# LuisaGroup/LuisaRender

Hardware: AMD Instinct MI355X
Metric: Msamples/s (+ fraction of HBM roofline) at fixed SPP, 1/2/4/8 GPU (higher is better)
Workload: dtype f32; 1 GPU; Contemporary Bathroom-class (procedural stand-in, ~600k tris), 1024x1024, 1024spp, depth 16; integrator=MegaPath, sampler=Independent (seed 19980810), spp=1024, parallelism=single GPU, collective=none (single GPU), scheduler=path pool, two contexts per lane (megapool_kernel.h)

## Files before the change

### __graft_entry__.py

```python
import os
import subprocess
import sys

ROOT = os.path.dirname(os.path.abspath(__file__))
if ROOT not in sys.path:
    sys.path.insert(0, ROOT)


def build() -> None:
    jobs = f"-j{min(os.cpu_count() or 4, 16)}"
    subprocess.check_call(["make", "-C", ROOT, jobs, "host", "oracle", "hip", "cli", "ieee", "shallow", "noearly", "nopair", "noride"])
    if os.path.isdir("/root/reference/src"):
        subprocess.check_call(["make", "-C", ROOT, jobs, "ref"])
    import luisarender_amd
    from luisarender_amd import _ffi
    _ffi.host_lib()
    assert os.path.exists(os.path.join(ROOT, "luisarender_amd", "lib", "liblrhip.so"))


def smoke() -> None:
    import numpy as np
    from luisarender_amd import Scene
    from oracle.check import Oracle
    from luisarender_amd.render import MegaPathRenderer
    from luisarender_amd.scenes import cornell_box

    scene = Scene.from_string(cornell_box(resolution=64, spp=8))
    renderer = MegaPathRenderer(0)
    renderer.upload(scene)
    renderer.render(0, 8, counters=True, sync=True)
    gpu = renderer.download(converted=False)
    cpu, counters = Oracle(scene).render(0, 8)
    rel = float(np.abs(gpu[..., :3] - cpu[..., :3]).sum() / np.abs(cpu[..., :3]).sum())
    gc = renderer.counters()
# ... 11 lines not shown
```

### include/lrhip.h

```cpp
#ifndef LRHIP_H
#define LRHIP_H

#include "lr_scene.h"

#ifdef __cplusplus
extern "C" {
#endif

typedef struct lrhip_ctx lrhip_ctx;

#define LRHIP_OK 0
#define LRHIP_ERROR_INVALID (-1)
#define LRHIP_ERROR_DEVICE (-2)
#define LRHIP_ERROR_UNSUPPORTED (-3)

typedef struct lrhip_render_params {
    uint32_t spp_begin, spp_end;
    uint32_t tile_begin, tile_end, tile_stride;
    uint32_t flags;
    uint32_t balance_shards;
    float shutter_weight;
} lrhip_render_params;

#define LRHIP_RENDER_COUNTERS 1u
// ... 102 lines not shown
int lrhip_set_wavefront(lrhip_ctx *ctx, uint32_t mode, uint32_t slice_paths);

#define LRHIP_FEAT_POOL 4096u
int lrhip_set_scheduler(lrhip_ctx *ctx, uint32_t mode);
int lrhip_set_texture_storage(lrhip_ctx *ctx, uint32_t mode);
uint64_t lrhip_packed_texels(lrhip_ctx *ctx);

uint32_t lrhip_pool_auto_triangles(uint32_t max_depth, uint32_t scene_spp);

#define LRHIP_FAMILY_NONE 0u
#define LRHIP_FAMILY_LANE 1u
#define LRHIP_FAMILY_POOL 2u
#define LRHIP_FAMILY_WAVEFRONT 3u
#define LRHIP_FAMILY_AOV 4u
#define LRHIP_PLAN_FLAG_COUNTERS 1u
#define LRHIP_PLAN_FLAG_ENV_TREE 2u
#define LRHIP_PLAN_FLAG_PACKED_TEXELS 4u
#define LRHIP_PLAN_FLAG_WANTS_POOL 8u
#define LRHIP_PLAN_FLAG_FIXED_FITS 16u
#define LRHIP_PLAN_WORDS 8
int lrhip_plan_kernels(uint32_t features, uint32_t force_features, uint32_t flags, uint32_t sampler_kind, uint32_t wf_mode, uint32_t max_depth,
                       uint32_t out[LRHIP_PLAN_WORDS]);

const char *lrhip_last_error(void);

#ifdef __cplusplus
}
#endif
#endif
```

### luisarender_amd/_ffi.py

```python
from __future__ import annotations

import ctypes as C
import os

_ROOT = os.path.dirname(os.path.abspath(__file__))
REPO_ROOT = os.path.dirname(_ROOT)
LIB_DIR = os.path.join(_ROOT, "lib")

u32, u64, i32, f32 = C.c_uint32, C.c_uint64, C.c_int32, C.c_float


class Vertex(C.Structure):
    _fields_ = [(n, f32) for n in ("px", "py", "pz", "nx", "ny", "nz", "u", "v")]


class Triangle(C.Structure):
    _fields_ = [("i0", u32), ("i1", u32), ("i2", u32)]


class AliasEntry(C.Structure):
    _fields_ = [("prob", f32), ("alias", u32)]


class UInt4(C.Structure):
# ... 203 lines not shown
        lib.lrhip_film_download.argtypes = [C.c_void_p, C.c_void_p, C.c_int]
        lib.lrhip_get_counters.argtypes = [C.c_void_p, C.POINTER(HipCounters)]
        lib.lrhip_last_render_ms.restype = C.c_double
        lib.lrhip_last_render_ms.argtypes = [C.c_void_p]
        lib.lrhip_set_stream.argtypes = [C.c_void_p, C.c_void_p]
        lib.lrhip_last_variant.restype = C.c_uint32
        lib.lrhip_last_variant.argtypes = [C.c_void_p]
        lib.lrhip_set_diagnostics.argtypes = [C.c_void_p, C.c_uint32, C.c_double]
        lib.lrhip_set_wavefront.argtypes = [C.c_void_p, C.c_uint32, C.c_uint32]
        lib.lrhip_set_scheduler.argtypes = [C.c_void_p, C.c_uint32]
        lib.lrhip_set_texture_storage.argtypes = [C.c_void_p, C.c_uint32]
        lib.lrhip_packed_texels.restype = C.c_uint64
        lib.lrhip_packed_texels.argtypes = [C.c_void_p]
        lib.lrhip_aov_download.argtypes = [C.c_void_p, C.c_uint32, C.c_void_p]
        lib.lrhip_denoise_default_params.restype = None
        lib.lrhip_denoise_default_params.argtypes = [C.POINTER(DenoiseParams)]
        lib.lrhip_denoise.argtypes = [C.c_void_p, C.POINTER(DenoiseParams)] + [C.c_void_p] * 5
        lib.lrhip_aov_denoise.argtypes = [C.c_void_p, C.POINTER(DenoiseParams), C.c_uint32, C.c_uint32, C.c_void_p]
        lib.lrhip_last_denoise_ms.restype = C.c_double
        lib.lrhip_last_denoise_ms.argtypes = [C.c_void_p]
        lib.lrhip_trace_rays.argtypes = [C.c_void_p, C.POINTER(RayQueryParams)]
        lib.lrhip_last_trace_ms.restype = C.c_double
        lib.lrhip_last_trace_ms.argtypes = [C.c_void_p]
        lib._lr_ready = True
    return lib
```

### luisarender_amd/csrc/hip/dev_scene.h

```cpp
#pragma once
#include "../../../include/lr_scene.h"
#include "dev_math.h"

namespace lrd {

struct alignas(16) DInstance {
    uint32_t handle[4];
    float c0[3]; uint32_t vertex_offset;
    float c1[3]; uint32_t triangle_offset;
    float c2[3]; uint32_t pad0;
    float t[3];  uint32_t pad1;
    float n0[3]; uint32_t pad2;
    float n1[3]; uint32_t pad3;
    float n2[3]; uint32_t pad4;
};
static_assert(sizeof(DInstance) == 128, "DInstance must be one cache line");

struct alignas(16) DClosure {
    uint32_t kind;
    uint32_t dynamic;
    float alpha_x, alpha_y;
    float c0[3]; float s0;
    float c1[3]; float s1;
    float c2[3]; float s2;
// ... 51 lines not shown
    const float *pdf;
    float direction[3];
    float cos_half_angle;
    uint32_t visible, constant_emission;
    uint32_t kind;
    float child_scale[2];
    uint32_t tree;
    const DEnvironment *child[2];
};

enum : uint32_t { kEnvNone = 0u, kEnvConstant = 1u, kEnvImage = 2u, kEnvDirectional = 3u, kEnvCombined = 4u };

struct DShadeTri {
    float p0[3];  uint32_t flags;
    float e1[3];  uint32_t tags;
    float e2[3];  uint32_t offset_bits;
    float n0[3];  float uv0x;
    float n1[3];  float uv0y;
    float n2[3];  float uv1x;
    float uv1y, uv2x, uv2y, tri_pdf;
    uint32_t inst, prim, tri_offset, pad;
};
static_assert(sizeof(DShadeTri) == 128, "one line per triangle");

constexpr uint32_t kWfKinds = 3u;
constexpr uint32_t kWfHeavyWords = 14u;
constexpr uint32_t kWfContWords = 25u;
constexpr uint32_t kWfSamplerWordsMax = 4u;
#ifndef LR_WF_ITEM
#define LR_WF_ITEM 1024
#endif
constexpr uint32_t kWfItemRecords = LR_WF_ITEM;
enum : uint32_t { kWfCountHeavy = 0u, kWfCountCont = 3u, kWfWorkCont = 4u, kWfWorkHeavy = 5u, kWfCounterWords = 8u,
                  kWfCarry = 8u, kWfCounterBufferWords = 12u };
struct WfArgs {
    uint32_t *heavy;
    uint32_t *cont;
    uint32_t *counts;
    uint32_t capacity;
    unsigned long long *accum;
    float accum_scale;
    uint32_t count_at_flush;
};

struct DScene {
    const DNodeQ *nodes;
// ... 19 lines not shown
    const lr_medium *media;
    uint32_t env_medium_tag;
    uint32_t integrator_kind, integrator_flags;
    float rr_threshold, env_prob;
    uint32_t light_count;
    uint32_t has_lights;
    uint32_t sampler_kind, seed;
    float film_clamp;
    uint32_t sampler_spp;
    uint32_t sobol_scale;
    float shutter_weight;
    uint32_t sampler_tile;
    uint32_t sampler_tile_jitter;
    const uint32_t *sobol_matrices;
    const uint32_t *sobol_bytes;
    const uint64_t *vdc_sobol, *vdc_sobol_inv;
    const uint64_t *vdc_bytes, *vdc_inv_bytes;
    const DEnvironment *env;
    WfArgs wf;
    float *aov;
    float *aov_partial;
    uint32_t aov_channels;
    uint32_t aov_offset[LR_AOV_COMPONENTS];
};

typedef const DScene __attribute__((address_space(4))) *DScenePtr;

struct DCounters {
    unsigned long long paths, closest_rays, shadow_rays, nodes_visited, tris_tested, surface_hits, nee_samples,
        path_length_sum, trace_steps, trace_steps_busy, shade_calls, shade_busy, trace_steps_starved, shade_cycles, trace_cycles, wave_cycles, nodes_empty,
        shade_light_cycles, shade_closure_cycles, shade_regen_cycles;
    unsigned long long probe[16];
};

struct RenderArgs {
    float4 *film;
    uint32_t spp_begin, spp_end;
    uint32_t tile_begin, tile_end, tile_stride;
    uint32_t tiles_x, tiles_y;
    uint32_t chunk_count;
    uint32_t item_count;
    uint32_t *work_counter;
    float4 *partial;
    uint32_t *spill;
    uint32_t total_threads;
    DCounters *counters;
// ... 32 lines not shown
```

### luisarender_amd/csrc/hip/dev_shade.h

```cpp
#pragma once
#include "dev_bsdf.h"
#include "dev_trace.h"

namespace lrd {


LR_HD uint32_t xxhash32_4(uint32_t x, uint32_t y, uint32_t z, uint32_t w) {
    constexpr uint32_t P2 = 2246822519u, P3 = 3266489917u, P4 = 668265263u, P5 = 374761393u;
    auto rot = [](uint32_t h) { return (h << 17u) | (h >> 15u); };
    auto h = w + P5 + x * P3;
    h = P4 * rot(h);
    h += y * P3;
    h = P4 * rot(h);
    h += z * P3;
    h = P4 * rot(h);
    h = P2 * (h ^ (h >> 15u));
    h = P3 * (h ^ (h >> 13u));
    return h ^ (h >> 16u);
}

LR_HD uint32_t xxhash32_1(uint32_t p) {
    constexpr uint32_t P2 = 2246822519u, P3 = 3266489917u, P4 = 668265263u, P5 = 374761393u;
    auto h = p + P5;
    h = P4 * ((h << 17u) | (h >> 15u));
// ... 582 lines not shown
    sp.tags = h.y;
    sp.offset_bits = h.w;
    sp.tri_offset = tri_offset;
    sp.uv = (sp.flags & LR_SHAPE_HAS_VERTEX_UV) ?
                f2{bary.x * uv0.x + bary.y * uv1.x + bary.z * uv2.x, bary.x * uv0.y + bary.y * uv1.y + bary.z * uv2.y} :
                f2{bary.y, bary.z};
    if (FULL) {
        auto r0 = ip[5], r1 = ip[6], r2 = ip[7];
        f3 n0 = mk3(a0.w, a1.x, a1.y), n1 = mk3(b0.w, b1.x, b1.y), n2 = mk3(c0.w, c1.x, c1.y);
        auto ns_local = bary.x * n0 + bary.y * n1 + bary.z * n2;
        f2 duv0{uv1.x - uv0.x, uv1.y - uv0.y}, duv1{uv2.x - uv0.x, uv2.y - uv0.y};
        auto det = duv0.x * duv1.y - duv0.y * duv1.x;
        auto inv_det = 1.f / det;
        auto dpdu_local = (dp0 * duv1.y - dp1 * duv0.y) * inv_det;
        auto fallback = frame_from_normal(sp.ng);
        auto dpdu = det == 0.f ? fallback.s : mul(dpdu_local);
        auto ns = (sp.flags & LR_SHAPE_HAS_VERTEX_NORMAL) ?
                      normalize(mk3(r0.x, r0.y, r0.z) * ns_local.x + mk3(r1.x, r1.y, r1.z) * ns_local.y + mk3(r2.x, r2.y, r2.z) * ns_local.z) :
                      sp.ng;
        sp.shading = frame_from_normal_tangent(face_forward(ns, sp.ng), dpdu);
    }
}

LR_D void reconstruct_baked(const DScene &scene, uint32_t tri, float u, float v, SurfacePoint &sp) {
    auto q = reinterpret_cast<const float4 *>(scene.shade_tris + tri);
    auto q0 = q[0], q1 = q[1], q2 = q[2], q3 = q[3], q4 = q[4], q5 = q[5], q6 = q[6];
    auto w = 1.f - u - v;
    f3 p0 = mk3(q0.x, q0.y, q0.z), e1 = mk3(q1.x, q1.y, q1.z), e2 = mk3(q2.x, q2.y, q2.z);
    sp.p = p0 + e1 * u + e2 * v;
    auto c = cross(e1, e2);
    sp.area = length(c) * .5f;
    sp.ng = normalize(c);
    sp.flags = __float_as_uint(q0.w);
    sp.tags = __float_as_uint(q1.w);
    sp.offset_bits = __float_as_uint(q2.w);
    sp.tri_offset = reinterpret_cast<const uint32_t *>(scene.shade_tris + tri)[30];
    f2 uv0{q3.w, q4.w}, uv1{q5.w, q6.x}, uv2{q6.y, q6.z};
    sp.uv = (sp.flags & LR_SHAPE_HAS_VERTEX_UV) ? f2{w * uv0.x + u * uv1.x + v * uv2.x, w * uv0.y + u * uv1.y + v * uv2.y} : f2{u, v};
    f2 duv0{uv1.x - uv0.x, uv1.y - uv0.y}, duv1{uv2.x - uv0.x, uv2.y - uv0.y};
    auto det = duv0.x * duv1.y - duv0.y * duv1.x;
    auto inv_det = 1.f / det;
    auto fallback = frame_from_normal(sp.ng);
    auto dpdu = det == 0.f ? fallback.s : (e1 * duv1.y - e2 * duv0.y) * inv_det;
    auto ns = (sp.flags & LR_SHAPE_HAS_VERTEX_NORMAL) ?
                  normalize(mk3(q3.x, q3.y, q3.z) * w + mk3(q4.x, q4.y, q4.z) * u + mk3(q5.x, q5.y, q5.z) * v) :
                  sp.ng;
    sp.shading = frame_from_normal_tangent(face_forward(ns, sp.ng), dpdu);
}



LR_D float surface_opacity(const DScene &scene, uint32_t tag, f2 uv) {
    auto one = [&](uint32_t t) {
        auto alpha_tex = scene.surfaces[t].raw.alpha_tex;
        return alpha_tex >= 0 ? texture_eval(scene, alpha_tex, uv).x : 1.f;
    };
    if (scene.surfaces[tag].raw.kind != LR_SURFACE_MIX) { return one(tag); }
    uint32_t stack[8];
    auto sp = 0u;
    stack[sp++] = tag;
    auto opacity = 1.f;
    while (sp > 0u) {
        const auto tag_here = stack[--sp];
        auto &s = scene.surfaces[tag_here].raw;
        if (s.kind == LR_SURFACE_MIX && sp + 2u <= 8u) { stack[sp++] = s.u[1], stack[sp++] = s.u[0]; }
        else { opacity *= one(tag_here); }
    }
    return opacity;
}

// ... 61 lines not shown
    auto n = front ? sp.ng : -sp.ng;
    return offset_ray_origin(sp.p, intersection_offset_factor(sp.offset_bits) * n);
}

LR_D void light_evaluate_with(const DScene &scene, const SurfacePoint &lp, float tri_pdf, f3 p_from, f3 &L, float &pdf);
LR_D void light_evaluate(const DScene &scene, const SurfacePoint &lp, uint32_t prim, f3 p_from, f3 &L, float &pdf) {
    light_evaluate_with(scene, lp, scene.tri_pdf[lp.tri_offset + prim], p_from, L, pdf);
}
LR_D void light_evaluate_with(const DScene &scene, const SurfacePoint &lp, float tri_pdf, f3 p_from, f3 &L, float &pdf) {
    auto &light = scene.lights[lp.tags & 4095u];
    auto pdf_area = tri_pdf / lp.area;
    auto cos_wo = abs_dot(normalize(p_from - lp.p), lp.ng);
    f3 Le = mk3(light.L[0], light.L[1], light.L[2]);
    if (light.dynamic) {
        auto v = texture_eval(scene, light.emission_tex, lp.uv);
        Le = max0(mk3(v.x, v.y, v.z)) * light.scale;
    }
    auto diff = lp.p - p_from;
    auto p = dot(diff, diff) * pdf_area * (1.0f / cos_wo);
    auto invalid = fabsf(cos_wo) < 1e-6f || (!light.two_sided && lp.back_facing);
    L = invalid ? mk3(0.f) : Le;
    pdf = invalid ? 0.f : p;
}


LR_D f3 mul3(const float *m, f3 v) { return mk3(m[0], m[1], m[2]) * v.x + mk3(m[3], m[4], m[5]) * v.y + mk3(m[6], m[7], m[8]) * v.z; }

struct EnvTables {
    const lr_texture *textures;
    const float *texels;
};
struct EnvEval {
    f3 L;
    float pdf;
};
struct EnvSample {
    f3 wi, L;
    float pdf;
};

LR_D f3 env_radiance(const EnvTables &tb, const DEnvironment &env, f2 uv) {
    auto v = texture_eval_tables(tb.textures, tb.texels, env.emission_tex, uv);
    auto rgb = env.constant_emission ? extend_rgb(v, tb.textures[env.emission_tex].channels) : mk3(v.x, v.y, v.z);
    return max0(rgb);
}
LR_D float env_directional_pdf(float p, float theta) {
    float sn, cs;
// ... 172 lines not shown
        return;
    }
    auto sa = env.child_scale[0], sb = env.child_scale[1];
    auto weight_a = sa / (sa + sb);
    auto first = u.x < weight_a;
    u.x = first ? u.x / weight_a : (u.x - weight_a) / (1.f - weight_a);
    auto s = env_sample_one(tb, env.child[first ? 0 : 1], u);
    auto o = env_evaluate_one(tb, env.child[first ? 1 : 0], s.wi);
    if (first) {
        L = s.L * sa + o.L * sb;
        pdf = lerp(s.pdf, o.pdf, 1.f - weight_a);
    } else {
        L = o.L * sa + s.L * sb;
        pdf = lerp(o.pdf, s.pdf, 1.f - weight_a);
    }
    wi = normalize(mul3(env.env_to_world, s.wi));
}

struct LightPick {
    Ray shadow;
    f3 L;
    float pdf;
};
template<bool ENV, bool NULL_SHAPE = false>
LR_D LightPick sample_one_light(const DScene &scene, const SurfacePoint &it, float u_light_selection, f2 u_light_surface) {
    LightPick out;
    out.L = mk3(0.f), out.pdf = 0.f;
    auto n = static_cast<float>(scene.light_count);
    auto is_env = false;
    auto tag = 0u;
    auto prob = 0.f;
    if (scene.env_prob == 1.f) {
        is_env = true, prob = 1.f;
    } else if (scene.env_prob == 0.f) {
        tag = static_cast<uint32_t>(clampf(u_light_selection * n, 0.f, n - 1.f)), prob = 1.f / n;
    } else {
        auto uu = (u_light_selection - scene.env_prob) / (1.f - scene.env_prob);
        tag = static_cast<uint32_t>(clampf(uu * n, 0.f, n - 1.f));
        is_env = u_light_selection < scene.env_prob;
        prob = is_env ? scene.env_prob : (1.f - scene.env_prob) / n;
    }
    if (is_env) {
        f3 wi;
        if (ENV && scene.env_kind != kEnvConstant) {
            env_sample(scene, u_light_surface, wi, out.L, out.pdf);
            out.pdf *= prob;
        } else {
            auto z = 1.0f - 2.0f * u_light_surface.x;
            auto r = sqrtf(fmaxf(1.0f - z * z, 0.0f));
            float sn, cs;
            sincos_2pi(u_light_surface.y, sn, cs);
            auto w = mk3(r * cs, r * sn, z);
            auto e = scene.env_to_world;
            wi = normalize(mk3(e[0], e[1], e[2]) * w.x + mk3(e[3], e[4], e[5]) * w.y + mk3(e[6], e[7], e[8]) * w.z);
            out.L = mk3(scene.env_L[0], scene.env_L[1], scene.env_L[2]);
            out.pdf = (kInvPi * 0.25f) * prob;
        }
        out.shadow.o = NULL_SHAPE ? it.p : robust_origin(it, wi);
        out.shadow.d = wi;
        out.shadow.t_min = 0.f, out.shadow.t_max = kFloatMax;
    } else {
        auto handle = scene.light_instances[tag];
        auto lh = reinterpret_cast<const uint4 *>(scene.instances + handle.instance_id)[0];
        auto l_tri_offset = scene.instances[handle.instance_id].triangle_offset;
        float u_remapped;
        auto slot = alias_slot(u_light_surface.x, lh.z, u_remapped);
        auto entry = scene.tri_alias[l_tri_offset + slot];
        auto pick = alias_pick(entry.prob, entry.alias, slot, u_remapped);
        f2 ut{pick.u, u_light_surface.y};
        f2 uvt = ut.x < ut.y ? f2{0.5f * ut.x, -0.5f * ut.x + ut.y} : f2{-0.5f * ut.y + ut.x, 0.5f * ut.y};
        SurfacePoint lp;
        reconstruct<false>(scene, handle.instance_id, pick.index, mk3(uvt.x, uvt.y, 1.0f - uvt.x - uvt.y), lp);
        lp.back_facing = dot(lp.ng, it.p - lp.p) < 0.f;
        light_evaluate(scene, lp, pick.index, it.p, out.L, out.pdf);
        out.pdf *= prob;
        auto p_from = NULL_SHAPE ? it.p : robust_origin(it, lp.p - it.p);
        auto Lv = lp.p - p_from;
        auto dist = length(Lv);
        out.shadow.o = p_from;
        out.shadow.d = Lv * (1.f / dist);
        out.shadow.t_min = 0.f, out.shadow.t_max = dist * .9999f;
    }
    return out;
// ... 4 lines not shown
```

### luisarender_amd/csrc/hip/lrhip_internal.h

```cpp
#pragma once
#include "../../../include/lrhip.h"

#include <hip/hip_runtime.h>

#include <algorithm>
#include <cmath>
#include <cstddef>
#include <cstring>
#include <string>
#include <vector>

#include "megapath_kernel.h"
#include "megapool_kernel.h"
#include "variants.h"

namespace lrh {

int fail(int code, const std::string &msg);

#define LR_HIP_CHECK(expr)                                                                                   \
    do {                                                                                                     \
        auto err_ = (expr);                                                                                  \
        if (err_ != hipSuccess) {                                                                            \
            return lrh::fail(LRHIP_ERROR_DEVICE, std::string{#expr} + ": " + hipGetErrorString(err_));       \
// ... 98 lines not shown
    hipEvent_t denoise_begin{nullptr}, denoise_end{nullptr};
    bool denoise_timed{false};
    lrh::DeviceBuffer raycast_rays, raycast_out;
    hipEvent_t raycast_begin{nullptr}, raycast_end{nullptr};
    double raycast_ms{0.};
    bool raycast_pending{false};
    int raycast_blocks[2]{-1, -1};
};

namespace lrh {

int kernel_blocks(lrhip_ctx *ctx, const KernelEntry &entry, unsigned lds_bytes, uint32_t &blocks_per_cu);

void release_scene(lrhip_ctx *ctx);

std::string validate_indices(const lr_scene *s);
constexpr uint64_t kByteTextureFloatBytes = 192ull << 20u;
std::vector<uint32_t> pack_byte_textures(const lr_scene *s, std::vector<lr_texture> &textures);
uint32_t bvh_depth(const lr_accel &accel);
std::vector<lrd::DNodeQ> build_packed_nodes(const lr_scene *s);
std::vector<uint8_t> build_padded_triangles(const lr_scene *s);
std::vector<lrd::DInstance> build_instances(const lr_scene *s);
std::vector<lrd::DShadeTri> build_shade_tris(const lr_scene *s, const std::vector<lrd::DInstance> &instances, std::string &error);
void set_camera(lrd::DScene &d, const lr_scene *s);

struct Chunking {
    uint32_t count, big_count, big, small;
};
Chunking chunking_of(uint32_t spp, double shard_tiles, double item_scale, bool taper);
int fixed_point_bits(float film_clamp, float shutter_weight, uint32_t spp);
int ensure_accum(lrhip_ctx *ctx, uint32_t pixel_count);
int ensure_pool(lrhip_ctx *ctx, uint32_t resident_blocks);
int render_wavefront(lrhip_ctx *ctx, const lrhip_render_params *p, const KernelPlan &plan, uint32_t tiles_x, uint32_t tiles_y,
                     uint32_t tiles_in_range, uint32_t tile_count);

hipError_t launch_resolve_partial(lrhip_ctx *ctx, const float4 *partial, uint32_t chunk_count, uint32_t tiles_x, uint32_t tile_begin,
                                  uint32_t tile_end, uint32_t tile_stride);
hipError_t launch_resolve_aov_partial(lrhip_ctx *ctx, uint32_t chunk_count, uint32_t tiles_x, uint32_t tile_begin, uint32_t tile_end,
                                      uint32_t tile_stride);
hipError_t launch_wf_resolve(lrhip_ctx *ctx, double inv_scale);
hipError_t launch_wf_carry(lrhip_ctx *ctx, uint32_t margin, uint32_t mode);

}
```

### luisarender_amd/csrc/hip/lrhip_tables.hip

```cpp
#include "lrhip_internal.h"

#include <limits>

namespace lrh {

namespace {
void normal_matrix(const float *m, float out[9]) {
    float a[3][3];
    for (auto c = 0; c < 3; c++) {
        for (auto r = 0; r < 3; r++) { a[c][r] = m[c * 4 + r]; }
    }
    auto one_over_det = 1.0f / (a[0][0] * (a[1][1] * a[2][2] - a[2][1] * a[1][2]) -
                                a[1][0] * (a[0][1] * a[2][2] - a[2][1] * a[0][2]) +
                                a[2][0] * (a[0][1] * a[1][2] - a[1][1] * a[0][2]));
    float inv[3][3];
    inv[0][0] = (a[1][1] * a[2][2] - a[2][1] * a[1][2]) * one_over_det;
    inv[0][1] = (a[2][1] * a[0][2] - a[0][1] * a[2][2]) * one_over_det;
    inv[0][2] = (a[0][1] * a[1][2] - a[1][1] * a[0][2]) * one_over_det;
    inv[1][0] = (a[2][0] * a[1][2] - a[1][0] * a[2][2]) * one_over_det;
    inv[1][1] = (a[0][0] * a[2][2] - a[2][0] * a[0][2]) * one_over_det;
    inv[1][2] = (a[1][0] * a[0][2] - a[0][0] * a[1][2]) * one_over_det;
    inv[2][0] = (a[1][0] * a[2][1] - a[2][0] * a[1][1]) * one_over_det;
    inv[2][1] = (a[2][0] * a[0][1] - a[0][0] * a[2][1]) * one_over_det;
    inv[2][2] = (a[0][0] * a[1][1] - a[1][0] * a[0][1]) * one_over_det;
// ... 106 lines not shown
        const lr_vertex *v[3] = {s->vertices + mesh.vertex_offset + tri.i0, s->vertices + mesh.vertex_offset + tri.i1,
            s->vertices + mesh.vertex_offset + tri.i2};
        auto &r = shade[i];
        std::memset(&r, 0, sizeof(r));
        for (auto c = 0; c < 3; c++) { r.p0[c] = bt.v0[c], r.e1[c] = bt.e1[c], r.e2[c] = bt.e2[c]; }
        float *n[3] = {r.n0, r.n1, r.n2};
        for (auto k = 0; k < 3; k++) {
            for (auto c = 0; c < 3; c++) { n[k][c] = di.n0[c] * v[k]->nx + di.n1[c] * v[k]->ny + di.n2[c] * v[k]->nz; }
        }
        r.uv0x = v[0]->u, r.uv0y = v[0]->v, r.uv1x = v[1]->u, r.uv1y = v[1]->v, r.uv2x = v[2]->u, r.uv2y = v[2]->v;
        r.flags = inst.handle.x & 1023u, r.tags = inst.handle.y, r.offset_bits = inst.handle.w;
        if ((r.flags & LR_SHAPE_HAS_SURFACE) != 0u) {
            const auto tag = (inst.handle.y >> 12u) & 4095u;
            if (tag < s->surface_count && s->surfaces[tag].kind >= LR_SURFACE_DISNEY) {
                r.flags |= (s->surfaces[tag].kind - LR_SURFACE_DISNEY + 1u) << 10u;
            }
        }
        r.tri_pdf = s->tri_pdf[mesh.triangle_offset + bt.prim];
        r.inst = bt.inst, r.prim = bt.prim, r.tri_offset = mesh.triangle_offset;
    }
    return shade;
}

void set_camera(lrd::DScene &d, const lr_scene *s) {
    auto &cam = d.camera;
    cam.kind = s->camera.kind, cam.width = s->camera.width, cam.height = s->camera.height;
    std::memcpy(cam.c2w, s->camera.camera_to_world, sizeof(cam.c2w));
    cam.tan_half_fov = s->camera.tan_half_fov, cam.focus_distance = s->camera.focus_distance;
    cam.lens_radius = s->camera.lens_radius, cam.projected_pixel_size = s->camera.projected_pixel_size;
    cam.ortho_scale = s->camera.ortho_scale, cam.clip_near = s->camera.clip_near, cam.clip_far = s->camera.clip_far;
}

std::vector<uint32_t> pack_byte_textures(const lr_scene *s, std::vector<lr_texture> &textures) {
    std::vector<uint32_t> packed;
    auto division_ok = true;
    for (auto b = 0u; b < 256u; b++) { division_ok = division_ok && lrd::byte_over_255(static_cast<float>(b)) == static_cast<float>(b) / 255.f; }
    for (auto &t : textures) {
        t.pad = 0u;
        const auto count = static_cast<uint64_t>(t.width) * t.height;
        if (t.kind != LR_TEX_IMAGE || count == 0u || t.texel_offset + count > s->texel_count) { continue; }
        const auto px = s->texels + t.texel_offset * 4u;
        bool same[4], product[4], quotient[4];
        for (auto c = 0u; c < 4u; c++) {
            same[c] = true, product[c] = true, quotient[c] = division_ok;
            for (uint64_t i = 0u; i < count && (same[c] || product[c] || quotient[c]); i++) {
                const auto v = px[i * 4u + c];
// ... 84 lines not shown
            d += 1u;
            return {};
        };
        for (uint32_t i = 0; i < s->environment_child_count; i++) {
            auto &c = s->environment_children[i];
            if (c.kind != LR_ENV_SPHERICAL && c.kind != LR_ENV_DIRECTIONAL && c.kind != LR_ENV_COMBINED) {
                return "environment child " + std::to_string(i) + ": invalid kind";
            }
            if (c.kind != LR_ENV_COMBINED && (c.emission_tex < 0 || static_cast<uint32_t>(c.emission_tex) >= s->texture_count)) {
                return "environment child " + std::to_string(i) + ": emission texture out of range";
            }
            if (auto bad = check_node(c, i, depth[i]); !bad.empty()) { return "environment child " + std::to_string(i) + ": " + bad; }
        }
        uint32_t root_depth = 0u;
        if (auto bad = check_node(s->environment, s->environment_child_count, root_depth); !bad.empty()) { return "environment: " + bad; }
        if (root_depth > static_cast<uint32_t>(LR_ENV_MAX_COMBINED_DEPTH)) {
            return "environment: Combined nodes nested deeper than LR_ENV_MAX_COMBINED_DEPTH";
        }
    }
    return {};
}

}
```

### luisarender_amd/csrc/hip/lrhip_upload.hip

```cpp
#include "lrhip_internal.h"

#include <array>
#include <functional>
#include <map>
#include <set>

using namespace lrh;

namespace {

template<typename T>
int upload(lrhip_ctx *ctx, const T *host, size_t count, const T **device) {
    DeviceBuffer b;
    b.bytes = std::max<size_t>(count * sizeof(T), 16u);
    LR_HIP_CHECK(hipMalloc(&b.ptr, b.bytes));
    ctx->scene_buffers.emplace_back(b);
    if (count != 0u) { LR_HIP_CHECK(hipMemcpy(b.ptr, host, count * sizeof(T), hipMemcpyHostToDevice)); }
    *device = static_cast<const T *>(b.ptr);
    return LRHIP_OK;
}

#define LR_UP(call)                                                    \
    if (auto rc_ = (call); rc_ != LRHIP_OK) { return rc_; }

// ... 309 lines not shown
    {
        auto packed = build_packed_nodes(s);
        LR_UP(upload(ctx, packed.data(), packed.size(), &d.nodes));
    }
    {
        auto padded = build_padded_triangles(s);
        const uint8_t *dev = nullptr;
        LR_UP(upload(ctx, padded.data(), padded.size(), &dev));
        d.bvh_tris = reinterpret_cast<const lr_bvh_triangle *>(dev);
    }
    LR_UP(upload(ctx, s->vertices, s->vertex_count, &d.vertices));
    LR_UP(upload(ctx, s->triangles, s->triangle_count, &d.triangles));
    LR_UP(upload(ctx, s->tri_alias, s->triangle_count, &d.tri_alias));
    LR_UP(upload(ctx, s->tri_pdf, s->triangle_count, &d.tri_pdf));
    LR_UP(upload(ctx, s->light_instances, s->light_instance_count, &d.light_instances));
    LR_UP(upload_textures(ctx, s));
    LR_UP(upload(ctx, &s->filter, 1u, &d.filter));
    auto instances = build_instances(s);
    LR_UP(upload(ctx, instances.data(), instances.size(), &d.instances));
    {
        std::string error;
        auto shade = build_shade_tris(s, instances, error);
        if (!error.empty()) { return fail(LRHIP_ERROR_INVALID, "lrhip_upload_scene: " + error); }
        LR_UP(upload(ctx, shade.data(), shade.size(), &d.shade_tris));
    }
    LR_UP(upload_surfaces(ctx, s));
    LR_UP(upload_lights(ctx, s));
    set_camera(d, s);
    LR_UP(upload_environment(ctx, s));
    d.max_depth = s->integrator.max_depth, d.rr_depth = s->integrator.rr_depth;
    d.integrator_kind = s->integrator.kind, d.integrator_flags = s->integrator.flags;
    if (s->integrator.kind > LR_INTEGRATOR_AOV) { return fail(LRHIP_ERROR_UNSUPPORTED, "lrhip_upload_scene: unknown integrator kind"); }
    d.env_medium_tag = s->integrator.environment_medium_tag;
    const auto nested = (ctx->features & lrd::kFeatNest) != 0u;
    if (s->integrator.kind == LR_INTEGRATOR_VPT_NAIVE) {
        for (uint32_t i = 0; i < s->instance_count; i++) {
            if ((s->instances[i].handle.x & LR_SHAPE_HAS_MEDIUM) && (s->instances[i].handle.y >> 24u) >= s->medium_count) {
                return fail(LRHIP_ERROR_INVALID, "lrhip_upload_scene: an instance references a medium that is not in scene->media");
            }
        }
        if (d.env_medium_tag != LR_INVALID_ID && d.env_medium_tag >= s->medium_count) {
            return fail(LRHIP_ERROR_INVALID, "lrhip_upload_scene: invalid environment medium tag");
        }
        if (auto r = upload(ctx, s->media, s->medium_count, &d.media); r != LRHIP_OK) { return r; }
        ctx->features = lrd::kFeatVpt;
        if (nested) {
            return fail(LRHIP_ERROR_UNSUPPORTED,
// ... 154 lines not shown
```

### luisarender_amd/csrc/hip/megapool_kernel.h

```cpp
#pragma once
#include "dev_wavefront.h"

namespace lrd {

#ifndef LR_MIN_WAVES
#define LR_MIN_WAVES 4
#endif
#ifndef LR_POOL_SHADE_LANES
#define LR_POOL_SHADE_LANES 56
#endif
#ifndef LR_POOL_IDLE_LANES
#define LR_POOL_IDLE_LANES 16
#endif
#ifndef LR_POOL_TURNOVER_LANES
#define LR_POOL_TURNOVER_LANES 12
#endif
#ifndef LR_POOL_PARK_ON_STACK
#define LR_POOL_PARK_ON_STACK 1
#endif
#ifndef LR_POOL_FUSED_FETCH
#define LR_POOL_FUSED_FETCH 1
#endif
#ifndef LR_POOL_FUSED_ALPHA
#define LR_POOL_FUSED_ALPHA 0
#endif
#ifndef LR_POOL_EARLY_FETCH
#define LR_POOL_EARLY_FETCH 1
#endif
#ifndef LR_POOL_LEAF_NODE_PAIR
#define LR_POOL_LEAF_NODE_PAIR 1
#endif
#ifndef LR_POOL_EARLY_TAIL_PRIO
#define LR_POOL_EARLY_TAIL_PRIO 3
#endif
#ifndef LR_POOL_STATE_LEAN
#define LR_POOL_STATE_LEAN 1
#endif
#ifndef LR_POOL_RAY_INIT
#define LR_POOL_RAY_INIT if (!mine)
#endif
#ifndef LR_POOL_SHADOW_RIDE
#define LR_POOL_SHADOW_RIDE 1
#endif
constexpr uint32_t kPoolSlots = 128u;

template<bool GENERIC>
constexpr uint32_t pool_quads() { return GENERIC ? 5u : 4u; }
constexpr uint32_t kPoolRecordQuadsMax = pool_quads<true>() + 1u;
constexpr uint32_t kPoolPending = 1u << 22u;

enum : uint32_t {
    kCtxShadow = 1u, kCtxClosest = 2u,
    kCtxHadShadow = 4u, kCtxHadClosest = 8u,
    kCtxDone = 16u,
    kCtxOccluded = 32u,
    kCtxSide = 64u,
    kCtxOpen = 128u,
};
struct PathCtx {
    f3 so, sd;
    float s_tmax;
    f3 no, nd;
    float n_tmin, n_tmax;
    uint32_t tri;
    float u, v;
// ... 198 lines not shown
            atomicAdd(&args.film[(PIXEL)].w, -1.f);                                                                                              \
        }                                                                                                                                        \
    } while (false)

template<uint32_t F>
__global__ __launch_bounds__(kBlockThreads, LR_MIN_WAVES) void megapool_kernel(DScenePtr scene_ptr, RenderArgs args) {
    const DScene &scene = *(const DScene *)scene_ptr;
    constexpr bool COUNT = (F & kFeatCount) != 0u, PCG = (F & kFeatGeneric) != 0u, ENV = (F & kFeatEnv) != 0u,
                   ALPHA = (F & kFeatAlpha) != 0u, DISNEY = (F & kFeatDisney) != 0u, WF = (F & kFeatWf) != 0u, CONT = (F & kFeatCont) != 0u;
    static_assert((F & kFeatPool) != 0u, "a pool variant");
    static_assert(kPoolParkedWords == 5u, "the shading block parks five words on top of a lane's stack (below): lrhip_upload_scene bounds the BVH depth with this constant");
    static_assert((F & (kFeatMix | kFeatLayered | kFeatAux | kFeatVpt | kFeatNest)) == 0u, "the pool scheduler exists for the lean kernels (closures inline)");
    static_assert(!WF || !DISNEY, "a wavefront variant is a lean kernel: the heavy closures live in heavy_kernel.h");
    static_assert(!CONT || WF, "the continuation pass exists in wavefront mode only");
    constexpr uint32_t SAMPLER_WORDS = PathSampler<PCG>::kSavedWords;
#ifdef LR_ONLY_SAMPLER
    constexpr bool PADDED = PCG && (LR_ONLY_SAMPLER) == LR_SAMPLER_PADDED_SOBOL;
#else
    constexpr bool PADDED = false;
#endif
    static_assert(PADDED == ((F & kFeatPadded) != 0u) || (F & kFeatPadded) == 0u, "a kFeatPadded kernel: generic sampler, LR_ONLY_SAMPLER = PaddedSobol");
    constexpr uint32_t QUADS = PADDED ? 4u : pool_quads<PCG>();
    constexpr bool RIDE = LR_POOL_SHADOW_RIDE != 0 && !WF;
    constexpr uint32_t RECORD = QUADS + (RIDE ? 1u : 0u);
    static_assert(RECORD <= kPoolRecordQuadsMax, "ensure_pool sizes the records");
    __shared__ uint32_t s_stack[kStackLds * kBlockThreads];
    __shared__ float4 s_stage[kWavesPerBlock * kStageWave];
#if LR_POOL_PARK_ON_STACK == 0
    __shared__ uint32_t s_park[5u * kBlockThreads];
    static_assert(kStackLds + 5u <= 16u, "the parking area is carved out of the round 1-3 stack: compile such pool variants with LR_STACK_LDS <= 11");
#endif
    __shared__ unsigned long long s_film[CONT ? 1u : kWavesPerBlock * 192u];
#ifdef LR_STALL_PROBE
    __shared__ uint32_t s_probe[kWavesPerBlock * kProbeWords];
    if ((threadIdx.x & 63u) < kProbeWords) { s_probe[(threadIdx.x >> 6u) * kProbeWords + (threadIdx.x & 63u)] = 0u; }
    const auto probe_wave = (F & kFeatCount) != 0u && (blockIdx.x % 9u) == 0u && __builtin_amdgcn_readfirstlane(threadIdx.x >> 6u) == ((blockIdx.x / 9u) & 3u);
#endif
    const auto tid = threadIdx.x;
    const auto lane = tid & 63u;
    const auto gtid = blockIdx.x * kBlockThreads + tid;
    const auto wave_in_block = __builtin_amdgcn_readfirstlane(tid >> 6u);
    TraversalStack stack{s_stack + tid, args.spill + gtid, args.total_threads, s_stage + wave_in_block * kStageWave};
    const auto film_tile = s_film + (CONT ? 0u : wave_in_block * 192u);
    const auto state_of = [&](uint32_t side, uint32_t quad) { return args.pool + static_cast<size_t>(side * RECORD + quad) * args.total_threads + gtid; };
    const auto state_load = [&](uint32_t side, uint32_t quad) { return *state_of(side, quad); };
    const auto state_store = [&](uint32_t side, uint32_t quad, float4 v) { *state_of(side, quad) = v; };
// ... 116 lines not shown
                    const auto q3 = state_load(side, 3u);
                    const auto depth = dp & 0xffffu;
                    const auto first_rr = scene.rr_depth == 0u ? 0u : scene.rr_depth - 1u;
                    const auto dimension = (scene.camera.kind == LR_CAMERA_THIN_LENS ? 4u : 2u) + 6u * depth + (depth > first_rr ? depth - first_rr : 0u) + 3u * stage;
                    uint32_t words[kWfSamplerWordsMax] = {__float_as_uint(q3.z), 0u, dimension, __float_as_uint(q3.w)};
                    sampler.restore(scene, words);
                    return;
                }
                const auto q3 = state_load(side, 3u);
                uint32_t words[kWfSamplerWordsMax] = {word0, __float_as_uint(q3.z), __float_as_uint(q3.w), __float_as_uint(state_load(side, QUADS - 1u).x)};
                sampler.restore(scene, words);
            };
            const auto sampler_leave = [&]() {
                if (PADDED) { return; }
                uint32_t words[kWfSamplerWordsMax] = {0u, 0u, 0u, 0u};
                sampler.save(words);
                word0 = words[0];
                state_store(side, 2u, make_float4(Li.x, Li.y, Li.z, __uint_as_float(words[0])));
                const auto q3 = state_load(side, 3u);
                state_store(side, 3u, make_float4(q3.x, q3.y, __uint_as_float(words[1]), __uint_as_float(words[2])));
                state_store(side, QUADS - 1u, make_float4(__uint_as_float(words[3]), 0.f, 0.f, 0.f));
            };
            auto sampler_left = false;
            if (path_open) {
                const auto q0 = state_load(side, 0u), q1 = state_load(side, 1u), q2 = state_load(side, 2u);
                nee = mk3(q0.x, q0.y, q0.z), pdf_bsdf = q0.w;
                beta = mk3(q1.x, q1.y, q1.z);
                const auto packed = __float_as_uint(q1.w);
                dp = packed & (RIDE ? 0x7fffffu : 0x3fffffu);
                Li = mk3(q2.x, q2.y, q2.z);
                word0 = __float_as_uint(q2.w);
                if (!LEAN_STATE) { load_ids(); }
                if (!PCG) {
                    uint32_t words[kWfSamplerWordsMax] = {word0, 0u, 0u, 0u};
                    sampler.restore(scene, words);
                }
            }
            auto want_shadow = false, want_closest = false;
            unsigned long long t_closure_sum = 0ull;
#ifdef LR_STALL_PROBE
            uint32_t t_lobe = 0u, t_eval = 0u, t_sample = 0u, t_hit = 0u, t_light = 0u;
            const auto probe_clock = []() { return static_cast<uint32_t>(__builtin_readcyclecounter()); };
            const auto t_block = probe_clock();
#endif
            auto park_kind = kInvalid;
            if (path_open) {
// ... 5 lines not shown
                    LR_POOL_FILM_ADD(Li, __float_as_uint(ids.x), __float_as_uint(ids.y), __float_as_uint(ids.z));
                    Li = mk3(0.f), nee = mk3(0.f);
                    dp &= ~kPoolPending;
                }
                if (traced_closest) {
                    if (COUNT) { local.shade_busy++; }
                    const auto wo = -rd;
                    const auto hit_valid = hit_tri != kInvalid;
                    auto u_light_selection = 0.f, u_lobe = 0.f, u_rr = 0.f;
                    f2 u_light_surface{0.f, 0.f}, u_bsdf{0.f, 0.f};
                    const auto rr = (dp & 0xffffu) + 1u >= scene.rr_depth;
                    if (!hit_valid && scene.env_kind != kEnvNone) {
                        f3 L = mk3(scene.env_L[0], scene.env_L[1], scene.env_L[2]);
                        auto pdf = kInvPi * 0.25f;
                        if (ENV && scene.env_kind != kEnvConstant) { env_evaluate(scene, rd, L, pdf); }
                        Li += beta * L * balance(pdf_bsdf, pdf * scene.env_prob);
                    }
                    SurfacePoint it;
                    auto has_surface = false;
#ifdef LR_STALL_PROBE
                    const auto t_h0 = probe_clock();
#endif
                    if (hit_valid) {
                        reconstruct_baked(scene, hit_tri, hit_u, hit_v, it);
                        it.back_facing = dot(wo, it.ng) < 0.0f;
                        if (COUNT) { local.surface_hits++; }
                        if (scene.has_lights && (it.flags & LR_SHAPE_HAS_LIGHT)) {
                            f3 L;
                            float pdf;
                            const auto prim = reinterpret_cast<const uint32_t *>(scene.shade_tris + hit_tri)[29];
                            light_evaluate(scene, it, prim, ro, L, pdf);
                            pdf *= (1.f - scene.env_prob) / static_cast<float>(scene.light_count);
                            Li += beta * L * balance(pdf_bsdf, pdf);
                        }
                        has_surface = (it.flags & LR_SHAPE_HAS_SURFACE) != 0u;
                    }
                    if (WF && has_surface) {
                        const auto heavy_kind = (it.flags >> 10u) & 3u;
                        if (heavy_kind != 0u) { park_kind = heavy_kind - 1u, has_surface = false; }
                    }
                    if (WF) {
                        if (lr_any(park_kind != kInvalid)) {
                            unsigned long long kind_mask[kWfKinds];
#pragma unroll
                            for (auto k = 0u; k < kWfKinds; k++) { kind_mask[k] = lr_ballot(park_kind == k); }
                            static_assert(kWfKinds == 3u, "three closure kinds");
                            const auto my_mask = park_kind == 0u ? kind_mask[0] : (park_kind == 1u ? kind_mask[1] : (park_kind == 2u ? kind_mask[2] : 0ull));
                            auto reserved = 0u;
                            if (my_mask != 0ull && lane == static_cast<uint32_t>(__ffsll(static_cast<long long>(my_mask))) - 1u) {
                                reserved = atomicAdd(scene.wf.counts + kWfCountHeavy + park_kind, static_cast<uint32_t>(__popcll(my_mask)));
                            }
#pragma unroll
                            for (auto k = 0u; k < kWfKinds; k++) {
                                const auto mask = kind_mask[k];
// ... 16 lines not shown
                            }
                        }
                    }
#ifdef LR_STALL_PROBE
                    asm volatile("" : "+v"(it.p.x), "+v"(it.ng.x), "+v"(Li.x));
                    const auto t_h1 = probe_clock();
                    t_hit = t_h1 - t_h0;
#endif
                    if (has_surface) {
                        if (COUNT) { local.path_length_sum++, local.nee_samples++; }
                        if constexpr (PADDED && LR_PADDED_DRAWS_OUT_OF_LINE != 0) {
                            sampler_take(0u);
                            const auto r = padded_draws(&scene, sampler.lo, sampler.w3, sampler.w2, false);
                            u_light_selection = r.a, u_light_surface = f2{r.b, r.c};
                        } else {
                            if (PCG) { sampler_take(0u); }
                            u_light_selection = sampler.next_1d();
                            u_light_surface = sampler.next_2d();
                            if (PCG) { sampler_leave(), sampler_left = !PADDED; }
                        }
#if LR_LIGHT_OUT_OF_LINE
                        const auto pick = sample_one_light_call<ENV>(&scene, it.p, it.ng, it.shading.n, it.offset_bits, u_light_selection, u_light_surface.x, u_light_surface.y);
#else
                        const auto pick = sample_one_light<ENV>(scene, it, u_light_selection, u_light_surface);
#endif
                        shadow = pick.shadow;
#ifdef LR_STALL_PROBE
                        asm volatile("" : "+v"(shadow.o.x), "+v"(shadow.d.x));
#endif
                        const auto t_closure = COUNT ? __builtin_readcyclecounter() : 0ull;
#ifdef LR_STALL_PROBE
                        t_light = static_cast<uint32_t>(t_closure) - t_h1;
#endif
                        const LobeTables tables{scene.closures, scene.surfaces, scene.textures, scene.texels};
                        DClosure closure;
                        Frame sh;
                        load_lobe(tables, it.uv, it.ng, wo, (it.tags >> 12u) & 4095u, it.shading, closure, sh);
#ifdef LR_STALL_PROBE
                        asm volatile("" : "+v"(closure.c0[0]), "+v"(closure.s0), "+v"(sh.n.x));
                        const auto t_l1 = probe_clock();
                        t_lobe = t_l1 - static_cast<uint32_t>(t_closure);
#endif
                        if (pick.pdf > 0.0f) {
                            const auto eval = closure_evaluate<DISNEY>(closure, sh, it.ng, wo, shadow.d);
                            const auto w = balance(pick.pdf, eval.pdf) / pick.pdf;
                            nee = w * beta * eval.f * pick.L;
                            want_shadow = nee.x != 0.f || nee.y != 0.f || nee.z != 0.f;
// ... 278 lines not shown
```

Measured before the change: 1287 Msamples/s.

## Hoist shade-triangle loads and sample lights from flattened per-triangle tables

The seven-quad baked shade-triangle record is now loaded up front, before the path-state loads, so its latency can overlap them. Hit reconstruction and emitted-light evaluation then reuse those registers instead of reloading from memory. Light sampling reads a new flattened table: per-light handles plus one 128-byte row per light triangle holding its three vertices and pdf. This replaces the chain of dependent instance, mesh and vertex lookups. The cost is extra registers for the hoisted quads, a wasted load for lanes that did not hit anything (they read triangle 0), a forced memory barrier, and the surface tri_offset now always being zero on this path.

```diff
diff --git a/__graft_entry__.py b/__graft_entry__.py
--- a/__graft_entry__.py
+++ b/__graft_entry__.py
@@ -9,7 +9,7 @@
 
 def build() -> None:
     jobs = f"-j{min(os.cpu_count() or 4, 16)}"
-    subprocess.check_call(["make", "-C", ROOT, jobs, "host", "oracle", "hip", "cli", "ieee", "shallow", "noearly", "nopair", "noride"])
+    subprocess.check_call(["make", "-C", ROOT, jobs, "host", "oracle", "hip", "cli", "ieee", "shallow", "noearly", "nopair", "noride", "noflat"])
     if os.path.isdir("/root/reference/src"):
         subprocess.check_call(["make", "-C", ROOT, jobs, "ref"])
     import luisarender_amd
diff --git a/include/lrhip.h b/include/lrhip.h
--- a/include/lrhip.h
+++ b/include/lrhip.h
@@ -1,5 +1,7 @@
 #ifndef LRHIP_H
 #define LRHIP_H
+
+#include <stddef.h>
 
 #include "lr_scene.h"
 
@@ -148,6 +150,8 @@
 int lrhip_plan_kernels(uint32_t features, uint32_t force_features, uint32_t flags, uint32_t sampler_kind, uint32_t wf_mode, uint32_t max_depth,
                        uint32_t out[LRHIP_PLAN_WORDS]);
 
+int lrhip_light_tables(const lr_scene *scene, void *handles, size_t handle_bytes, void *rows, size_t row_bytes, uint32_t counts[2]);
+
 const char *lrhip_last_error(void);
 
 #ifdef __cplusplus
diff --git a/luisarender_amd/_ffi.py b/luisarender_amd/_ffi.py
--- a/luisarender_amd/_ffi.py
+++ b/luisarender_amd/_ffi.py
@@ -249,5 +249,7 @@
         lib.lrhip_trace_rays.argtypes = [C.c_void_p, C.POINTER(RayQueryParams)]
         lib.lrhip_last_trace_ms.restype = C.c_double
         lib.lrhip_last_trace_ms.argtypes = [C.c_void_p]
+        if hasattr(lib, "lrhip_light_tables"):
+            lib.lrhip_light_tables.argtypes = [C.POINTER(Scene), C.c_void_p, C.c_size_t, C.c_void_p, C.c_size_t, C.POINTER(u32 * 2)]
         lib._lr_ready = True
     return lib
diff --git a/luisarender_amd/csrc/hip/dev_scene.h b/luisarender_amd/csrc/hip/dev_scene.h
--- a/luisarender_amd/csrc/hip/dev_scene.h
+++ b/luisarender_amd/csrc/hip/dev_scene.h
@@ -97,6 +97,20 @@
     uint32_t inst, prim, tri_offset, pad;
 };
 static_assert(sizeof(DShadeTri) == 128, "one line per triangle");
+
+struct alignas(16) DLightHandle {
+    uint32_t instance_id;
+    uint32_t triangle_offset;
+    uint32_t alias_count;
+    uint32_t first_row;
+};
+static_assert(sizeof(DLightHandle) == 16, "DLightHandle: one quad");
+struct alignas(128) DLightTri {
+    lr_vertex v[3];
+    float tri_pdf;
+    uint32_t pad[7];
+};
+static_assert(sizeof(DLightTri) == 128, "one line per light triangle");
 
 constexpr uint32_t kWfKinds = 3u;
 constexpr uint32_t kWfHeavyWords = 14u;
@@ -162,6 +176,8 @@
     float *aov_partial;
     uint32_t aov_channels;
     uint32_t aov_offset[LR_AOV_COMPONENTS];
+    const DLightHandle *light_handles;
+    const DLightTri *light_tris;
 };
 
 typedef const DScene __attribute__((address_space(4))) *DScenePtr;
diff --git a/luisarender_amd/csrc/hip/dev_shade.h b/luisarender_amd/csrc/hip/dev_shade.h
--- a/luisarender_amd/csrc/hip/dev_shade.h
+++ b/luisarender_amd/csrc/hip/dev_shade.h
@@ -628,9 +628,16 @@
     }
 }
 
-LR_D void reconstruct_baked(const DScene &scene, uint32_t tri, float u, float v, SurfacePoint &sp) {
+struct BakedQuads {
+    float4 q0, q1, q2, q3, q4, q5, q6;
+};
+LR_D BakedQuads baked_load(const DScene &scene, uint32_t tri) {
     auto q = reinterpret_cast<const float4 *>(scene.shade_tris + tri);
-    auto q0 = q[0], q1 = q[1], q2 = q[2], q3 = q[3], q4 = q[4], q5 = q[5], q6 = q[6];
+    return BakedQuads{q[0], q[1], q[2], q[3], q[4], q[5], q[6]};
+}
+template<typename TriOffset>
+LR_D void reconstruct_baked_compute(const BakedQuads &r, float u, float v, SurfacePoint &sp, TriOffset &&tri_offset) {
+    auto q0 = r.q0, q1 = r.q1, q2 = r.q2, q3 = r.q3, q4 = r.q4, q5 = r.q5, q6 = r.q6;
     auto w = 1.f - u - v;
     f3 p0 = mk3(q0.x, q0.y, q0.z), e1 = mk3(q1.x, q1.y, q1.z), e2 = mk3(q2.x, q2.y, q2.z);
     sp.p = p0 + e1 * u + e2 * v;
@@ -640,7 +647,7 @@
     sp.flags = __float_as_uint(q0.w);
     sp.tags = __float_as_uint(q1.w);
     sp.offset_bits = __float_as_uint(q2.w);
-    sp.tri_offset = reinterpret_cast<const uint32_t *>(scene.shade_tris + tri)[30];
+    sp.tri_offset = tri_offset();
     f2 uv0{q3.w, q4.w}, uv1{q5.w, q6.x}, uv2{q6.y, q6.z};
     sp.uv = (sp.flags & LR_SHAPE_HAS_VERTEX_UV) ? f2{w * uv0.x + u * uv1.x + v * uv2.x, w * uv0.y + u * uv1.y + v * uv2.y} : f2{u, v};
     f2 duv0{uv1.x - uv0.x, uv1.y - uv0.y}, duv1{uv2.x - uv0.x, uv2.y - uv0.y};
@@ -652,6 +659,29 @@
                   normalize(mk3(q3.x, q3.y, q3.z) * w + mk3(q4.x, q4.y, q4.z) * u + mk3(q5.x, q5.y, q5.z) * v) :
                   sp.ng;
     sp.shading = frame_from_normal_tangent(face_forward(ns, sp.ng), dpdu);
+}
+LR_D void reconstruct_baked(const DScene &scene, uint32_t tri, float u, float v, SurfacePoint &sp) {
+    reconstruct_baked_compute(baked_load(scene, tri), u, v, sp, [&]() { return reinterpret_cast<const uint32_t *>(scene.shade_tris + tri)[30]; });
+}
+
+LR_D void reconstruct_light_point(uint4 h, float4 q0, float4 q1, float4 q2, float4 q3, float4 a0, float4 a1, float4 b0, float4 b1, float4 c0, float4 c1,
+                                  f3 bary, SurfacePoint &sp) {
+    f3 m0 = mk3(q0.x, q0.y, q0.z), m1 = mk3(q1.x, q1.y, q1.z), m2 = mk3(q2.x, q2.y, q2.z), mt = mk3(q3.x, q3.y, q3.z);
+    auto mul = [&](f3 v) { return m0 * v.x + m1 * v.y + m2 * v.z; };
+    f3 p0 = mk3(a0.x, a0.y, a0.z), p1 = mk3(b0.x, b0.y, b0.z), p2 = mk3(c0.x, c0.y, c0.z);
+    f2 uv0{a1.z, a1.w}, uv1{b1.z, b1.w}, uv2{c1.z, c1.w};
+    auto dp0 = p1 - p0, dp1 = p2 - p0;
+    sp.p = mul(bary.x * p0 + bary.y * p1 + bary.z * p2) + mt;
+    auto c = cross(mul(dp0), mul(dp1));
+    sp.area = length(c) * .5f;
+    sp.ng = normalize(c);
+    sp.flags = h.x & 1023u;
+    sp.tags = h.y;
+    sp.offset_bits = h.w;
+    sp.tri_offset = __float_as_uint(q1.w);
+    sp.uv = (sp.flags & LR_SHAPE_HAS_VERTEX_UV) ?
+                f2{bary.x * uv0.x + bary.y * uv1.x + bary.z * uv2.x, bary.x * uv0.y + bary.y * uv1.y + bary.z * uv2.y} :
+                f2{bary.y, bary.z};
 }
 
 
@@ -759,7 +789,6 @@
     L = invalid ? mk3(0.f) : Le;
     pdf = invalid ? 0.f : p;
 }
-
 
 LR_D f3 mul3(const float *m, f3 v) { return mk3(m[0], m[1], m[2]) * v.x + mk3(m[3], m[4], m[5]) * v.y + mk3(m[6], m[7], m[8]) * v.z; }
 
@@ -978,7 +1007,7 @@
     f3 L;
     float pdf;
 };
-template<bool ENV, bool NULL_SHAPE = false>
+template<bool ENV, bool NULL_SHAPE = false, bool FLAT = false>
 LR_D LightPick sample_one_light(const DScene &scene, const SurfacePoint &it, float u_light_selection, f2 u_light_surface) {
     LightPick out;
     out.L = mk3(0.f), out.pdf = 0.f;
@@ -1015,6 +1044,31 @@
         out.shadow.o = NULL_SHAPE ? it.p : robust_origin(it, wi);
         out.shadow.d = wi;
         out.shadow.t_min = 0.f, out.shadow.t_max = kFloatMax;
+    } else if (FLAT) {
+        const auto handle = *reinterpret_cast<const uint4 *>(scene.light_handles + tag);
+        float u_remapped;
+        auto slot = alias_slot(u_light_surface.x, handle.z, u_remapped);
+        auto entry = scene.tri_alias[handle.y + slot];
+        auto ip = reinterpret_cast<const float4 *>(scene.instances + handle.x);
+        auto lh = reinterpret_cast<const uint4 *>(ip)[0];
+        auto q0 = ip[1], q1 = ip[2], q2 = ip[3], q3 = ip[4];
+        auto pick = alias_pick(entry.prob, entry.alias, slot, u_remapped);
+        const auto row = reinterpret_cast<const float4 *>(scene.light_tris + (handle.w + pick.index));
+        auto a0 = row[0], a1 = row[1], b0 = row[2], b1 = row[3], c0 = row[4], c1 = row[5];
+        const auto tri_pdf = reinterpret_cast<const float *>(row)[24];
+        f2 ut{pick.u, u_light_surface.y};
+        f2 uvt = ut.x < ut.y ? f2{0.5f * ut.x, -0.5f * ut.x + ut.y} : f2{-0.5f * ut.y + ut.x, 0.5f * ut.y};
+        SurfacePoint lp;
+        reconstruct_light_point(lh, q0, q1, q2, q3, a0, a1, b0, b1, c0, c1, mk3(uvt.x, uvt.y, 1.0f - uvt.x - uvt.y), lp);
+        lp.back_facing = dot(lp.ng, it.p - lp.p) < 0.f;
+        light_evaluate_with(scene, lp, tri_pdf, it.p, out.L, out.pdf);
+        out.pdf *= prob;
+        auto p_from = NULL_SHAPE ? it.p : robust_origin(it, lp.p - it.p);
+        auto Lv = lp.p - p_from;
+        auto dist = length(Lv);
+        out.shadow.o = p_from;
+        out.shadow.d = Lv * (1.f / dist);
+        out.shadow.t_min = 0.f, out.shadow.t_max = dist * .9999f;
     } else {
         auto handle = scene.light_instances[tag];
         auto lh = reinterpret_cast<const uint4 *>(scene.instances + handle.instance_id)[0];
diff --git a/luisarender_amd/csrc/hip/lrhip_internal.h b/luisarender_amd/csrc/hip/lrhip_internal.h
--- a/luisarender_amd/csrc/hip/lrhip_internal.h
+++ b/luisarender_amd/csrc/hip/lrhip_internal.h
@@ -144,6 +144,11 @@
 std::vector<uint8_t> build_padded_triangles(const lr_scene *s);
 std::vector<lrd::DInstance> build_instances(const lr_scene *s);
 std::vector<lrd::DShadeTri> build_shade_tris(const lr_scene *s, const std::vector<lrd::DInstance> &instances, std::string &error);
+struct LightTables {
+    std::vector<lrd::DLightHandle> handles;
+    std::vector<lrd::DLightTri> rows;
+};
+LightTables build_light_tables(const lr_scene *s, std::string &error);
 void set_camera(lrd::DScene &d, const lr_scene *s);
 
 struct Chunking {
diff --git a/luisarender_amd/csrc/hip/lrhip_tables.hip b/luisarender_amd/csrc/hip/lrhip_tables.hip
--- a/luisarender_amd/csrc/hip/lrhip_tables.hip
+++ b/luisarender_amd/csrc/hip/lrhip_tables.hip
@@ -152,6 +152,47 @@
     return shade;
 }
 
+LightTables build_light_tables(const lr_scene *s, std::string &error) {
+    LightTables out;
+    std::vector<uint32_t> first_row(s->mesh_count, LR_INVALID_ID);
+    out.handles.resize(s->light_instance_count);
+    for (uint32_t i = 0; i < s->light_instance_count; i++) {
+        const auto id = s->light_instances[i].instance_id;
+        if (id >= s->instance_count) { error = "light instance references an unknown instance"; return {}; }
+        const auto &h = s->instances[id].handle;
+        const auto mesh_index = h.x >> 10u;
+        if (mesh_index >= s->mesh_count) { error = "light instance references an unknown mesh"; return {}; }
+        const auto &mesh = s->meshes[mesh_index];
+        if (first_row[mesh_index] == LR_INVALID_ID) {
+            if (static_cast<uint64_t>(mesh.triangle_offset) + mesh.triangle_count > s->triangle_count ||
+                static_cast<uint64_t>(mesh.vertex_offset) + mesh.vertex_count > s->vertex_count ||
+                out.rows.size() + mesh.triangle_count >= LR_INVALID_ID) {
+                error = "light mesh beyond the triangle or vertex table";
+                return {};
+            }
+            first_row[mesh_index] = static_cast<uint32_t>(out.rows.size());
+            for (uint32_t p = 0; p < mesh.triangle_count; p++) {
+                const auto tri = s->triangles[mesh.triangle_offset + p];
+                if (tri.i0 >= mesh.vertex_count || tri.i1 >= mesh.vertex_count || tri.i2 >= mesh.vertex_count) {
+                    error = "light triangle references an unknown vertex";
+                    return {};
+                }
+                lrd::DLightTri row;
+                std::memset(&row, 0, sizeof(row));
+                row.v[0] = s->vertices[mesh.vertex_offset + tri.i0], row.v[1] = s->vertices[mesh.vertex_offset + tri.i1];
+                row.v[2] = s->vertices[mesh.vertex_offset + tri.i2];
+                row.tri_pdf = s->tri_pdf[mesh.triangle_offset + p];
+                out.rows.push_back(row);
+            }
+        }
+        auto &dst = out.handles[i];
+        std::memset(&dst, 0, sizeof(dst));
+        dst.instance_id = id, dst.triangle_offset = mesh.triangle_offset, dst.alias_count = h.z;
+        dst.first_row = first_row[mesh_index];
+    }
+    return out;
+}
+
 void set_camera(lrd::DScene &d, const lr_scene *s) {
     auto &cam = d.camera;
     cam.kind = s->camera.kind, cam.width = s->camera.width, cam.height = s->camera.height;
@@ -282,3 +323,18 @@
 }
 
 }
+
+extern "C" int lrhip_light_tables(const lr_scene *scene, void *handles, size_t handle_bytes, void *rows, size_t row_bytes, uint32_t counts[2]) {
+    if (scene == nullptr || counts == nullptr) { return lrh::fail(LRHIP_ERROR_INVALID, "lrhip_light_tables: NULL argument"); }
+    std::string error;
+    const auto tables = lrh::build_light_tables(scene, error);
+    if (!error.empty()) { return lrh::fail(LRHIP_ERROR_INVALID, "lrhip_light_tables: " + error); }
+    counts[0] = static_cast<uint32_t>(tables.handles.size()), counts[1] = static_cast<uint32_t>(tables.rows.size());
+    const auto want_handles = tables.handles.size() * sizeof(lrd::DLightHandle), want_rows = tables.rows.size() * sizeof(lrd::DLightTri);
+    if ((handles != nullptr && handle_bytes < want_handles) || (rows != nullptr && row_bytes < want_rows)) {
+        return lrh::fail(LRHIP_ERROR_INVALID, "lrhip_light_tables: buffer too small");
+    }
+    if (handles != nullptr && want_handles != 0u) { std::memcpy(handles, tables.handles.data(), want_handles); }
+    if (rows != nullptr && want_rows != 0u) { std::memcpy(rows, tables.rows.data(), want_rows); }
+    return LRHIP_OK;
+}
diff --git a/luisarender_amd/csrc/hip/lrhip_upload.hip b/luisarender_amd/csrc/hip/lrhip_upload.hip
--- a/luisarender_amd/csrc/hip/lrhip_upload.hip
+++ b/luisarender_amd/csrc/hip/lrhip_upload.hip
@@ -355,7 +355,15 @@
         std::string error;
         auto shade = build_shade_tris(s, instances, error);
         if (!error.empty()) { return fail(LRHIP_ERROR_INVALID, "lrhip_upload_scene: " + error); }
+        if (shade.empty()) { shade.resize(1u), std::memset(shade.data(), 0, sizeof(shade[0])); }
         LR_UP(upload(ctx, shade.data(), shade.size(), &d.shade_tris));
+    }
+    {
+        std::string error;
+        const auto light_tables = build_light_tables(s, error);
+        if (!error.empty()) { return fail(LRHIP_ERROR_INVALID, "lrhip_upload_scene: " + error); }
+        LR_UP(upload(ctx, light_tables.handles.data(), light_tables.handles.size(), &d.light_handles));
+        LR_UP(upload(ctx, light_tables.rows.data(), light_tables.rows.size(), &d.light_tris));
     }
     LR_UP(upload_surfaces(ctx, s));
     LR_UP(upload_lights(ctx, s));
diff --git a/luisarender_amd/csrc/hip/megapool_kernel.h b/luisarender_amd/csrc/hip/megapool_kernel.h
--- a/luisarender_amd/csrc/hip/megapool_kernel.h
+++ b/luisarender_amd/csrc/hip/megapool_kernel.h
@@ -41,6 +41,15 @@
 #endif
 #ifndef LR_POOL_SHADOW_RIDE
 #define LR_POOL_SHADOW_RIDE 1
+#endif
+#ifndef LR_SHADE_FLAT_LOADS
+#define LR_SHADE_FLAT_LOADS 1
+#endif
+#ifndef LR_SHADE_FLAT_JOINT
+#define LR_SHADE_FLAT_JOINT LR_SHADE_FLAT_LOADS
+#endif
+#ifndef LR_SHADE_FLAT_LIGHT
+#define LR_SHADE_FLAT_LIGHT LR_SHADE_FLAT_LOADS
 #endif
 constexpr uint32_t kPoolSlots = 128u;
 
@@ -285,6 +294,8 @@
     static_assert(PADDED == ((F & kFeatPadded) != 0u) || (F & kFeatPadded) == 0u, "a kFeatPadded kernel: generic sampler, LR_ONLY_SAMPLER = PaddedSobol");
     constexpr uint32_t QUADS = PADDED ? 4u : pool_quads<PCG>();
     constexpr bool RIDE = LR_POOL_SHADOW_RIDE != 0 && !WF;
+    constexpr bool FLAT = LR_SHADE_FLAT_JOINT != 0 && !WF;
+    constexpr bool FLAT_LIGHT = LR_SHADE_FLAT_LIGHT != 0 && !WF && LR_LIGHT_OUT_OF_LINE == 0;
     constexpr uint32_t RECORD = QUADS + (RIDE ? 1u : 0u);
     static_assert(RECORD <= kPoolRecordQuadsMax, "ensure_pool sizes the records");
     __shared__ uint32_t s_stack[kStackLds * kBlockThreads];
@@ -447,6 +458,11 @@
                 state_store(side, QUADS - 1u, make_float4(__uint_as_float(words[3]), 0.f, 0.f, 0.f));
             };
             auto sampler_left = false;
+            BakedQuads hq;
+            if (FLAT) {
+                hq = baked_load(scene, traced_closest && hit_tri != kInvalid ? hit_tri : 0u);
+                asm volatile("" ::: "memory");
+            }
             if (path_open) {
                 const auto q0 = state_load(side, 0u), q1 = state_load(side, 1u), q2 = state_load(side, 2u);
                 nee = mk3(q0.x, q0.y, q0.z), pdf_bsdf = q0.w;
@@ -498,14 +514,19 @@
                     const auto t_h0 = probe_clock();
 #endif
                     if (hit_valid) {
-                        reconstruct_baked(scene, hit_tri, hit_u, hit_v, it);
+                        if (FLAT) { reconstruct_baked_compute(hq, hit_u, hit_v, it, []() { return 0u; }); }
+                        else { reconstruct_baked(scene, hit_tri, hit_u, hit_v, it); }
                         it.back_facing = dot(wo, it.ng) < 0.0f;
                         if (COUNT) { local.surface_hits++; }
                         if (scene.has_lights && (it.flags & LR_SHAPE_HAS_LIGHT)) {
                             f3 L;
                             float pdf;
-                            const auto prim = reinterpret_cast<const uint32_t *>(scene.shade_tris + hit_tri)[29];
-                            light_evaluate(scene, it, prim, ro, L, pdf);
+                            if (FLAT) {
+                                light_evaluate_with(scene, it, hq.q6.w, ro, L, pdf);
+                            } else {
+                                const auto prim = reinterpret_cast<const uint32_t *>(scene.shade_tris + hit_tri)[29];
+                                light_evaluate(scene, it, prim, ro, L, pdf);
+                            }
                             pdf *= (1.f - scene.env_prob) / static_cast<float>(scene.light_count);
                             Li += beta * L * balance(pdf_bsdf, pdf);
                         }
@@ -568,7 +589,7 @@
 #if LR_LIGHT_OUT_OF_LINE
                         const auto pick = sample_one_light_call<ENV>(&scene, it.p, it.ng, it.shading.n, it.offset_bits, u_light_selection, u_light_surface.x, u_light_surface.y);
 #else
-                        const auto pick = sample_one_light<ENV>(scene, it, u_light_selection, u_light_surface);
+                        const auto pick = sample_one_light<ENV, false, FLAT_LIGHT>(scene, it, u_light_selection, u_light_surface);
 #endif
                         shadow = pick.shadow;
 #ifdef LR_STALL_PROBE
```

Result: no change. 1290 Msamples/s, median of 6 (+0.2%).
